# AVianEco/Softspoken

Measured on AMD Instinct MI355X. Metric: audio-seconds processed/sec (whole node), 16 kHz mono, higher is better.
Workload: dtype f16x2

## Files before the change

### softspoken_amd/build.py

```python
from __future__ import annotations

import os
import subprocess
import sys

HERE = os.path.dirname(os.path.abspath(__file__))
CSRC = os.path.join(HERE, "csrc")
OBJ = os.path.join(CSRC, "_obj")
LIB = os.path.join(HERE, "libsoftspoken_hip.so")
DEV_LIB = os.path.join(HERE, "libsoftspoken_hip_dev.so")
SOURCES = ["conv2.hip", "conv2_ups.hip", "conv4.hip", "conv4_ups.hip", "conv1s.hip", "conv9s.hip", "frontend.hip", "heads.hip", "weights.hip", "engine.hip", "host.hip", "abi.hip", "stream.hip", "separate.hip"]
HEADERS = [os.path.join(CSRC, h) for h in ("kernels.h", "engine.h", "dsp.h", "mfma_util.h", "conv4_forms.h", "stream16.h")] + [os.path.join(os.path.dirname(HERE), "include", "softspoken.h")]
FLAGS = ["-O3", "--offload-arch=gfx950", "-fPIC", "-std=c++17", "-Wno-unused-value"]
EXTRA_FLAGS = {"frontend.hip": ["-fno-slp-vectorize"], "conv4.hip": ["-fno-slp-vectorize"], "conv4_ups.hip": ["-fno-slp-vectorize"],
               "conv1s.hip": ["-fno-slp-vectorize"], "conv9s.hip": ["-fno-slp-vectorize"]}
DEV_SOURCES = ("conv2.hip", "conv2_ups.hip", "conv4.hip", "conv4_ups.hip", "conv1s.hip", "frontend.hip", "engine.hip", "weights.hip", "abi.hip", "separate.hip")
JITTER_LIB = DEV_LIB


def _hipcc():
    for cand in (os.environ.get("HIPCC"), "/opt/rocm/bin/hipcc"):
        if cand and os.path.exists(cand):
            return cand
    return "hipcc"


def _stale(target, deps):
    if not os.path.exists(target):
        return True
    t = os.path.getmtime(target)
    return any(os.path.getmtime(d) > t for d in deps)


def build(force: bool = False, verbose: bool = True, dev: bool = False, jitter: bool = False) -> str:
    dev = dev or jitter
    os.makedirs(OBJ, exist_ok=True)
    hipcc = _hipcc()
    objs, procs = [], []
# ... 28 lines not shown
```

### softspoken_amd/csrc/conv9s.hip

```cpp
#include "kernels.h"
#include "stream16.h"
#include <algorithm>

namespace ss {

static constexpr int kProjFrag = 2 * 2 * 2 * 1024;
static constexpr uint32_t kRowB = kW * 64, kRowB8 = (kW / 2) * 64;

__global__ __launch_bounds__(64 * kS1Waves) __attribute__((amdgpu_waves_per_eu(2, 2)))
void conv9_stream16_kernel(ConvArgs a, int rows_per_unit, int total_units) {
    extern __shared__ __attribute__((aligned(16))) char smem[];
    char* sW = smem;
    char* sP = smem + 2 * kBank;

    const int tid = threadIdx.x, lane = tid & 63, wave = __builtin_amdgcn_readfirstlane(tid >> 6);
    const int g = lane >> 4, c = lane & 15;
    for (int p = tid; p < 2 * kBank / 16; p += 64 * kS1Waves) *(u32x4*)(sW + p * 16) = *(const u32x4*)((const char*)a.wpk + (size_t)p * 16);
    for (int p = tid; p < kProjFrag / 16; p += 64 * kS1Waves) *(u32x4*)(sP + p * 16) = *(const u32x4*)((const char*)a.proj_w + (size_t)p * 16);
    const f32x4 bias[2] = {*(const f32x4*)(a.bias + 8 * g), *(const f32x4*)(a.bias + 8 * g + 4)};
    __syncthreads();

    const char* wl_base = sW + lane * 16;
    const char* pl_base = sP + lane * 16;
    const char* fw_base = (const char*)a.flat_w4 + lane * 16;
    const int bands = kH / rows_per_unit;
    const int64_t lo = a.lo_delta;
    uint32_t ovf = 0;

    for (int unit = (int)blockIdx.x * kS1Waves + wave; unit < total_units; unit += (int)gridDim.x * kS1Waves) {
        const int s = unit % kStrips, b = (unit / kStrips) % bands, n = unit / (kStrips * bands);
        const int x0 = kStripCols * s - 1, y0 = b * rows_per_unit, ylast = y0 + rows_per_unit - 1;
        uint32_t keep[2], voff[2]; bool st_lane[2];
        int xt[2];
#pragma unroll
        for (int t = 0; t < 2; ++t) {
            const int mm = 2 * c + t;
            xt[t] = x0 + mm;
            keep[t] = (unsigned)xt[t] < (unsigned)kW ? 0xffffffffu : 0u;
            st_lane[t] = mm >= 1 && mm <= kStripCols && xt[t] < kW;
            voff[t] = (uint32_t)min(max(xt[t], 0), kW - 1) * 64u + (uint32_t)g * 16u;
        }
        const uint32_t voff8 = (uint32_t)(min(max(xt[1], 0), kW - 1) >> 1) * 64u + (uint32_t)g * 16u;
        const char* hw = (const char*)a.src0 + (size_t)n * kH * kRowB;
        const char* c1w = (const char*)a.xp0 + (size_t)n * kH * kRowB;
        const char* c8w = (const char*)a.xp1 + (size_t)n * (kH / 2) * kRowB8;
        char* ow = (char*)a.out + (size_t)n * kH * kRowB;

        auto load_row = [&](S16Row& H, int r) {
            const char* p = hw + (size_t)min(max(r, 0), kH - 1) * kRowB;
#pragma unroll
            for (int t = 0; t < 2; ++t) { H.f[t][0] = *(const u32x4*)(p + voff[t]); H.f[t][1] = *(const u32x4*)(p + lo + voff[t]); }
        };
        auto mask_row = [&](S16Row& H, int r) {
            const uint32_t rk = (unsigned)r < (unsigned)kH ? 0xffffffffu : 0u;
#pragma unroll
            for (int t = 0; t < 2; ++t)
#pragma unroll
                for (int pq = 0; pq < 2; ++pq)
#pragma unroll
                    for (int e = 0; e < 4; ++e) H.f[t][pq][e] &= keep[t] & rk;
        };
        S16Row H0, H1, H2;
        S16Row C1;
        u32x4 C8[2];
        auto load_c1 = [&](int r) {
            const char* p = c1w + (size_t)r * kRowB;
#pragma unroll
            for (int t = 0; t < 2; ++t) { C1.f[t][0] = *(const u32x4*)(p + voff[t]); C1.f[t][1] = *(const u32x4*)(p + lo + voff[t]); }
        };
        auto load_c8 = [&](int r8) {
            const char* p = c8w + (size_t)r8 * kRowB8;
            C8[0] = *(const u32x4*)(p + voff8); C8[1] = *(const u32x4*)(p + lo + voff8);
        };
        f32x4 F[2] = {f32x4{0.f, 0.f, 0.f, 0.f}, f32x4{0.f, 0.f, 0.f, 0.f}};
        uint32_t ovt[2] = {0u, 0u};

        auto row_step = [&](int y, S16Row& Ha, const S16Row& Hb, S16Row& Hn) {
            S16Ring ring;
            ring.rd(wl_base, 0);
            u32x4 pw[2][2][2];
#pragma unroll
            for (int q = 0; q < 8; ++q) pw[q >> 2][(q >> 1) & 1][q & 1] = *(const u32x4*)(pl_base + q * 1024);
            const u32x4 fwh = *(const u32x4*)(fw_base + (size_t)(2 * y) * 1024), fwl = *(const u32x4*)(fw_base + (size_t)(2 * y + 1) * 1024);
            __builtin_amdgcn_sched_barrier(0);
            f32x4 P[3][2][2];
#pragma unroll
            for (int t = 0; t < 2; ++t)
#pragma unroll
                for (int u = 0; u < 2; ++u) { P[0][t][u] = f32x4{0.f, 0.f, 0.f, 0.f}; P[1][t][u] = bias[u]; P[2][t][u] = f32x4{0.f, 0.f, 0.f, 0.f}; }
            u32x4 c8t0[2];
#pragma unroll
            for (int pq = 0; pq < 2; ++pq)
#pragma unroll
                for (int e = 0; e < 4; ++e) c8t0[pq][e] = (uint32_t)s16_shr1((int)C8[pq][e]);
#pragma unroll
            for (int src = 0; src < 2; ++src)
#pragma unroll
                for (int pr = 0; pr < 3; ++pr)
#pragma unroll
                    for (int u = 0; u < 2; ++u)
#pragma unroll
                        for (int t = 0; t < 2; ++t) {
                            const int pq = pr == 0 ? 1 : 0;
                            const u32x4& x = src == 0 ? C1.f[t][pq] : (t ? C8[pq] : c8t0[pq]);
                            P[1][t][u] = s16_mfma(pw[src][u][pr == 1 ? 1 : 0], x, P[1][t][u]);
                        }
            __builtin_amdgcn_sched_barrier(0);
            load_c1(min(y + 1, ylast));
            load_c8(min(y + 1, ylast) >> 1);
            __builtin_amdgcn_sched_barrier(0);
            s16_taps(ring, wl_base, Ha, Hb, Hn, P, [&](int tap) {
                if (tap == 2) load_row(Ha, min(y + 2, ylast + 1));
                if (tap == 5) mask_row(Hn, y + 1);
            });
            float v[2][2][4];
            s16_combine(P, v);
            uint32_t kh[2][4], kl[2][4];
#pragma unroll
            for (int t = 0; t < 2; ++t) {
                s16_split_px(v[t], kh[t], kl[t]);
#pragma unroll
                for (int i = 0; i < 4; ++i) ovt[t] = pk_max_u16(ovt[t], kh[t][i]);
            }
#pragma unroll
            for (int pr = 0; pr < 3; ++pr)
#pragma unroll
                for (int t = 0; t < 2; ++t) {
                    const uint32_t (&k)[4] = pr == 0 ? kl[t] : kh[t];
                    F[t] = s16_mfma(pr == 1 ? fwl : fwh, u32x4{k[0], k[1], k[2], k[3]}, F[t]);
                }
            if (a.store_out) {
                char* p = ow + (size_t)y * kRowB;
#pragma unroll
                for (int t = 0; t < 2; ++t)
                    if (st_lane[t]) {
                        *(u32x4*)(p + voff[t]) = u32x4{kh[t][0], kh[t][1], kh[t][2], kh[t][3]};
                        *(u32x4*)(p + lo + voff[t]) = u32x4{kl[t][0], kl[t][1], kl[t][2], kl[t][3]};
                    }
            }
        };

        load_row(H0, y0 - 1); load_row(H1, y0); load_c1(y0); load_c8(y0 >> 1); load_row(H2, y0 + 1);
        mask_row(H0, y0 - 1); mask_row(H1, y0);
        int k = 0;
        for (; k + 3 <= rows_per_unit; k += 3) {
            row_step(y0 + k, H0, H1, H2);
            row_step(y0 + k + 1, H1, H2, H0);
            row_step(y0 + k + 2, H2, H0, H1);
        }
        if (k < rows_per_unit) {
            row_step(y0 + k, H0, H1, H2);
            if (k + 1 < rows_per_unit) row_step(y0 + k + 1, H1, H2, H0);
        }
#pragma unroll
        for (int t = 0; t < 2; ++t) {
            if (g == 0 && st_lane[t]) {
                float* fp = a.flat_part + ((size_t)n * bands + b) * 4 * kW + xt[t];
#pragma unroll
                for (int r = 0; r < 4; ++r) fp[r * kW] = F[t][r];
            }
            if (st_lane[t]) ovf = pk_max_u16(ovf, ovt[t]);
        }
    }
    if (((ovf & 0x7fff7fffu) + 0x04000400u) & 0x80008000u) atomicOr(a.range_flag, 1);
}

static bool px64(ActStride s) { return s.pix == 64u; }
bool conv9_stream_supports(const ConvArgs& a) {
    return a.H == kH && a.W == kW && a.Cout == kC && a.C0 == kC && a.C1 == 0 && a.C0x == kC && a.C1x == kC && a.src0 && a.xp0 && a.xp1 && a.wpk &&
           a.proj_w && a.bias && a.flat_w4 && a.flat_part && (a.out || !a.store_out) && !a.pool_out && !a.res_in && a.lo_delta != 0 && a.range_flag &&
           a.N > 0 && px64(a.s_src0) && px64(a.s_xp0) && px64(a.s_xp1) && (px64(a.s_out) || !a.store_out);
}
const char* conv9_stream_variant() { return "conv9_stream16_kernel"; }
size_t conv9_stream_proj_bytes() { return kProjFrag; }
size_t conv9_stream_flat_bytes() { return (size_t)kH * 2 * 1024; }
bool conv9_stream_rows_ok(int rows_per_unit) { return rows_per_unit >= 2 && !(rows_per_unit & 1) && kH % rows_per_unit == 0 && rows_per_unit <= kMaxRows; }
int conv9_stream_flat_groups(int rows_per_unit) { return kH / rows_per_unit; }
double conv9_stream_issued_macs(int N) { return (double)N * kH * kStrips * ((24 + 108 + 6) / 3) * (16.0 * 16 * 32); }

hipError_t launch_conv9_stream(const ConvArgs& a, int rows_per_unit, int grid_override, int num_cus, hipStream_t s) {
    if (!conv9_stream_supports(a) || !conv9_stream_rows_ok(rows_per_unit)) return hipErrorInvalidValue;
    const int64_t total = (int64_t)a.N * (kH / rows_per_unit) * kStrips;
    if (total >= (int64_t)1 << 30) return hipErrorInvalidValue;
    const int cus = num_cus > 0 ? num_cus : 256;
    int grid = (int)std::min<int64_t>(cus, (total + kS1Waves - 1) / kS1Waves);
    if (grid_override > 0) grid = std::min(grid, grid_override);
    static std::atomic<uint64_t> attr_done{0};
    const size_t lds = 2 * (size_t)kBank + kProjFrag;
    if (hipError_t e = allow_full_lds((const void*)conv9_stream16_kernel, attr_done)) return e;
    hipLaunchKernelGGL(conv9_stream16_kernel, dim3(grid), dim3(64 * kS1Waves), lds, s, a, rows_per_unit, (int)total);
    return hipGetLastError();
}

}
```

### softspoken_amd/csrc/engine.h

```cpp
#pragma once
#include "../../include/softspoken.h"
#include "kernels.h"

#include <map>
#include <set>
#include <string>
#include <vector>

namespace ss {

inline size_t pcm_bytes_per_sample(int format) {
    switch (format) {
        case SS_PCM_U8: case SS_PCM_S8: return 1;
        case SS_PCM_S16: case SS_PCM_S16BE: return 2;
        case SS_PCM_S24: case SS_PCM_S24BE: return 3;
        case SS_PCM_F64: case SS_PCM_F64BE: return 8;
        default: return 4;
    }
}

int fail(ss_ctx* c, int code, const std::string& msg);
const char* thread_error();

#define HIPCHK(c, expr)                                                                                   \
// ... 5 lines not shown

struct BlobEntry { char name[96]; uint32_t dtype, ndim; int64_t shape[4]; uint64_t offset, nbytes; };
static_assert(sizeof(BlobEntry) == 152, "blob entry layout");
struct Blob {
    std::map<std::string, BlobEntry> e;
    const char* base = nullptr;
    size_t size = 0;
    bool has(const std::string& k) const { return e.count(k) != 0; }
    const float* f32(const std::string& k, size_t count, std::string& err) const;
};
bool parse_blob(const void* p, size_t n, Blob& b, std::string& err);

enum Precision { kFp32 = 0, kBf16 = 1, kF16x2 = 2 };

struct ConvPlan {
    std::string name;
    void* d_w2 = nullptr; float* d_bias2 = nullptr; float* d_res_bias = nullptr; float* d_rank1 = nullptr;
    void* d_w3 = nullptr; void* d_proj = nullptr; float* d_bias3 = nullptr;
    void* d_w_ups = nullptr;
    bool s1_range_proven = false;
    void* d_w_s1 = nullptr;
    void* d_w_s16 = nullptr;
    void* d_proj_s16 = nullptr;
    void* d_w_upsr = nullptr;
    void* d_w_ups32 = nullptr;
    int ups32_nt = 1;
    int Cout = 0, NT = 1, C0 = 0, C1 = 0, R0 = 0, R1 = 0, H = 0, W = 0;
};

struct FileRec {
    int64_t off = 0;
    int64_t n = 0;
    int64_t n_padded = 0;
    double duration = 0;
    int64_t W = 0, win_base = 0;
    int64_t bin_off = 0; int n_bins = 0;
};

struct StreamSet;
struct SepState;

struct SepPlan {
    int N = 0, hop = 0;
    int64_t W = 0, n_bins = 0, windows_run = 0;
    std::vector<ss_separation_range> ranges;
};
// ... 170 lines not shown
```

### softspoken_amd/csrc/engine.hip

```cpp
#include "engine.h"

#include <algorithm>
#include <chrono>
#include <cmath>
#include <cstdio>
#include <cstdlib>
#include <cstring>

namespace ss {

static thread_local std::string g_err;

int fail(ss_ctx* c, int code, const std::string& msg) {
    g_err = msg;
    if (c) c->err = msg;
    return code;
}
const char* thread_error() { return g_err.c_str(); }

double now_ms() { return std::chrono::duration<double, std::milli>(std::chrono::steady_clock::now().time_since_epoch()).count(); }

static int stat_id(ss_ctx* c, const std::string& name) {
    for (size_t i = 0; i < c->stats.size(); ++i) if (c->stats[i].name == name) return (int)i;
    KStat k; k.name = name; c->stats.push_back(k);
// ... 262 lines not shown
    a.N = n; a.H = pa.H; a.W = pa.W; a.Cout = pa.Cout; a.C0 = pa.C0; a.C1 = pa.C1; a.relu = 1;
    b.src0 = h; b.wpk = pb.d_w2; b.bias = pb.d_bias3; b.out = out; b.pool_out = pool;
    b.N = n; b.H = pb.H; b.W = pb.W; b.Cout = pb.Cout; b.C0 = pb.Cout; b.C1 = 0; b.relu = 1;
    b.proj_w = pb.d_proj; b.xp0 = x0; b.xp1 = x1; b.C0x = pa.C0; b.C1x = pa.C1;
    b.flat_w4 = ex.flat_w4; b.flat_part = ex.flat_part; b.store_out = ex.store_out;
    a.dbg = b.dbg = base_dbg();
    if (!(stride_of(ws, x0, a.s_src0) && stride_of(ws, x1, a.s_src1) && stride_of(ws, h, a.s_out) && stride_of(ws, h, b.s_src0) &&
          stride_of(ws, out, b.s_out) && stride_of(ws, pool, b.s_pool)))
        return fail(c, SS_ERR_STATE, "no byte order for a tensor of " + pa.name);
    b.s_xp0 = a.s_src0; b.s_xp1 = a.s_src1;
    ConvArgs au = a;
    au.wpk = pa.d_w_ups;
    const bool ups = c->prec == kF16x2 && pa.d_w_ups && x1 && conv_ups_supports(au, cus);
    if ((!ups && !conv_v4_supports(a, pa.NT, cus, prec4)) || !conv_v4_supports(b, pb.NT, cus, prec4)) return 1;
    mark_written(c, ws, h); mark_written(c, ws, pool);
    if (ex.store_out) mark_written(c, ws, out);
    const double px = (double)n * pa.H * pa.W, cin = pa.C0 + pa.C1, cinb = pa.C0 + pa.C1 / 4.0;
    const double flops_a = 2.0 * px * pa.Cout * 9.0 * cin, bytes_a = px * es * (cinb + pa.Cout);
    auto v4 = [&](const ConvPlan& p, ConvArgs& x, double flops, double bytes) {
        return conv_launch(c, stream, conv_v4_variant(x, p.NT, cus, prec4), p.name, x, flops, bytes, -1.0,
                           [&](ConvArgs& y) { return launch_conv3x3_v4(y, p.NT, cus, prec4, stream); });
    };
    int rc;
    if (ups) {
        ScopedLaunch sl(c, stream, std::string(conv_ups_variant()) + "/" + pa.name, flops_a, bytes_a, px * pa.Cout * (9.0 * pa.C0 + 4.0 * pa.C1));
        HIPCHK(c, launch_conv3x3_ups(au, cus, stream));
    } else if ((rc = v4(pa, a, flops_a, bytes_a))) return rc;
    const double flops_b = 2.0 * px * pb.Cout * (9.0 * pb.Cout + cin) + (ex.flat_part ? 2.0 * px * 32 * 4 : 0.0);
    const double bytes_b = px * es * (pb.Cout + cinb + (ex.flat_part && !ex.store_out ? 0 : pb.Cout) + (pool ? pb.Cout / 4.0 : 0));
    if (c->prec == kF16x2 && ex.flat_part && ex.flat_rows && pb.d_w_s16 && pb.d_proj_s16 && dev_env("SOFTSPOKEN_C9S", 1)) {
        ConvArgs bs = b;
        bs.wpk = pb.d_w_s16; bs.proj_w = pb.d_proj_s16; bs.flat_w4 = ex.flat_rows;
        const int rows = dev_env("SOFTSPOKEN_C9S_ROWS", 32);
        if (conv9_stream_supports(bs) && conv9_stream_rows_ok(rows)) {
            const int grid = dev_env("SOFTSPOKEN_C9S_GRID", 0);
            if ((rc = conv_launch(c, stream, conv9_stream_variant(), pb.name, bs, flops_b, bytes_b, conv9_stream_issued_macs(n),
                                  [&](ConvArgs& y) { return launch_conv9_stream(y, rows, grid, cus, stream); })))
                return rc;
            ws.flat_groups = conv9_stream_flat_groups(rows);
            return SS_OK;
        }
    }
    if ((rc = v4(pb, b, flops_b, bytes_b))) return rc;
    if (ex.flat_part) ws.flat_groups = conv_v4_flat_groups();
    return SS_OK;
}

// ... 403 lines not shown
```

### softspoken_amd/csrc/kernels.h

```cpp
#pragma once
#include <hip/hip_runtime.h>
#include <stdint.h>
#include <atomic>
#include <cstdlib>

namespace ss {

#ifdef SS_DEVBUILD
static inline int dev_env(const char* name, int dflt) { const char* v = getenv(name); return v ? atoi(v) : dflt; }
#else
static constexpr int dev_env(const char*, int dflt) { return dflt; }
#endif

inline hipError_t allow_full_lds(const void* kernel, std::atomic<uint64_t>& done) {
    int dev = 0;
    hipError_t e = hipGetDevice(&dev);
    if (e != hipSuccess) return e;
    const uint64_t bit = 1ull << (dev & 63);
    if (done.load(std::memory_order_acquire) & bit) return hipSuccess;
    e = hipFuncSetAttribute(kernel, hipFuncAttributeMaxDynamicSharedMemorySize, 160 * 1024);
    if (e == hipSuccess) done.fetch_or(bit, std::memory_order_release);
    return e;
}

// ... 95 lines not shown
const char* conv_upsr_variant();
size_t conv_upsr_weight_bytes(int C0, int C1, int Cout);
hipError_t launch_conv3x3_upsr(const ConvArgs& a, int num_cus, hipStream_t s);

bool conv_ups32_supports(const ConvArgs& a, int NT, int MTW, int num_cus);
const char* conv_ups32_variant(int NT, int MTW);
size_t conv_ups32_weight_bytes(int C0, int C1, int Cout);
hipError_t launch_conv3x3_ups32(const ConvArgs& a, int NT, int MTW, int num_cus, hipStream_t s);

bool conv1_stream_supports(const ConvArgs& a);
const char* conv1_stream_variant(const ConvArgs& a, int form);
size_t conv1_stream_weight_bytes();
hipError_t launch_conv1_stream(const ConvArgs& a, int form, int rows_per_unit, int num_cus, hipStream_t s);

bool conv9_stream_supports(const ConvArgs& a);
const char* conv9_stream_variant();
size_t conv9_stream_proj_bytes();
size_t conv9_stream_flat_bytes();
bool conv9_stream_rows_ok(int rows_per_unit);
int conv9_stream_flat_groups(int rows_per_unit);
double conv9_stream_issued_macs(int N);
hipError_t launch_conv9_stream(const ConvArgs& a, int rows_per_unit, int grid_override, int num_cus, hipStream_t s);

struct Head1dWeights { float w1[4][4][3], b1[4], w2[4][4][3], wr[4][4], b2r[4], wo[4], bo, fscale; };
hipError_t launch_mask_head_parts(const float* parts, int n_parts, const float* flat_bias, const Head1dWeights& hw, float* logits,
                                  int N, hipStream_t s);
hipError_t launch_spec_tail(const void* x, int64_t lo_delta, const float* w , const float* bias, float* spec, int N, int prec,
                            hipStream_t s);

static constexpr int kMelLo = 10, kMelHi = 32, kMelPitch = 43;
struct FrontendTables {
    const float4* pretw;
    const float2* w2048;
    const int* mel_start;
    const int* mel_count;
    const int* mel_off;
    const float* mel_w;
    int mel_nw;
    const float* mel_wp;
    int dbg;
    const float2* win2;
    const float2* twt;
    const float2* wkt;
    const float* mel_wq;
    const int* mel_p0;
};
// ... 50 lines not shown
```

### softspoken_amd/csrc/stream16.h

```cpp
#pragma once
#include "mfma_util.h"

namespace ss {

static constexpr int kH = 128, kW = 256, kC = 32;
static constexpr int kStrips = 9, kStripCols = 30;
static constexpr int kBank = 9 * 2 * 1024;
static constexpr int kS1Waves = 8;
static constexpr int kMaxRows = 32;

struct S16Row { u32x4 f[2][2]; };

__device__ __forceinline__ f32x4 s16_mfma(const u32x4& a, const u32x4& b, const f32x4& c) {
    return __builtin_amdgcn_mfma_f32_16x16x32_f16(__builtin_bit_cast(f16x8, a), __builtin_bit_cast(f16x8, b), c, 0, 0, 0);
}
__device__ __forceinline__ int s16_shr1(int v) { return __builtin_amdgcn_update_dpp(0, v, 0x111, 0xf, 0xf, true); }
__device__ __forceinline__ int s16_shl1(int v) { return __builtin_amdgcn_update_dpp(0, v, 0x101, 0xf, 0xf, true); }
__device__ __forceinline__ float s16_shr1f(float v) { return __int_as_float(s16_shr1(__float_as_int(v))); }
__device__ __forceinline__ float s16_shl1f(float v) { return __int_as_float(s16_shl1(__float_as_int(v))); }

struct S16Ring {
    u32x4 wh[2][2], wl[2][2];
    __device__ __forceinline__ void rd(const char* wl_base, int tap) {
#pragma unroll
// ... 16 lines not shown
#pragma unroll
        for (int pr = 0; pr < 3; ++pr)
#pragma unroll
            for (int u = 0; u < 2; ++u)
#pragma unroll
                for (int t = 0; t < 2; ++t)
                    P[dx][t][u] = s16_mfma(pr == 1 ? ring.wl[tap & 1][u] : ring.wh[tap & 1][u], Hr.f[t][pr == 0 ? 1 : 0], P[dx][t][u]);
        __builtin_amdgcn_sched_barrier(0);
        if (tap + 1 < 9) after_tap(tap);
    }
    __builtin_amdgcn_sched_barrier(0);
}

__device__ __forceinline__ void s16_combine(const f32x4 (&P)[3][2][2], float (&v)[2][2][4]) {
#pragma unroll
    for (int u = 0; u < 2; ++u)
#pragma unroll
        for (int r = 0; r < 4; ++r) {
            v[0][u][r] = relu_i(P[1][0][u][r] + s16_shr1f(P[0][1][u][r]) + P[2][1][u][r]);
            v[1][u][r] = relu_i(P[1][1][u][r] + P[0][0][u][r] + s16_shl1f(P[2][0][u][r]));
        }
}

__device__ __forceinline__ void s16_split_px(const float (&val)[2][4], uint32_t (&kh)[4], uint32_t (&kl)[4]) {
#pragma unroll
    for (int i = 0; i < 4; ++i) {
        const float e0 = val[i >> 1][2 * (i & 1)], e1 = val[i >> 1][2 * (i & 1) + 1];
        kh[i] = pack_f16(e0, e1);
        kl[i] = split_lo(kh[i], e0, e1);
    }
}

}
```

### softspoken_amd/csrc/weights.hip

```cpp
#include "engine.h"

#include <algorithm>
#include <cmath>
#include <cstring>

namespace ss {

const float* Blob::f32(const std::string& k, size_t count, std::string& err) const {
    auto it = e.find(k);
    if (it == e.end()) { err = "weights blob: missing tensor '" + k + "'"; return nullptr; }
    if (it->second.dtype != 0 || it->second.nbytes != count * 4) {
        err = "weights blob: tensor '" + k + "' has wrong dtype/size"; return nullptr;
    }
    return (const float*)(base + it->second.offset);
}

bool parse_blob(const void* p, size_t n, Blob& b, std::string& err) {
    if (n < 16 || memcmp(p, "SSWBLOB1", 8) != 0) { err = "weights blob: bad magic"; return false; }
    uint32_t cnt; memcpy(&cnt, (const char*)p + 8, 4);
    if (16 + (size_t)cnt * sizeof(BlobEntry) > n) { err = "weights blob: truncated table"; return false; }
    b.base = (const char*)p; b.size = n;
    for (uint32_t i = 0; i < cnt; ++i) {
        BlobEntry en; memcpy(&en, (const char*)p + 16 + (size_t)i * sizeof(BlobEntry), sizeof(BlobEntry));
        en.name[95] = 0;
// ... 186 lines not shown
                for (int l = 0; l < 64; ++l)
                    for (int e = 0; e < 8; ++e) {
                        const int co = l & 31, k = ci * 32 + s * 16 + (l >> 5) * 8 + e;
                        const size_t off = (size_t)ci * 2 * bank_r + (size_t)t * 2048 + ((size_t)s * 64 + l) * 16 + (size_t)e * 2;
                        put(off, off + bank_r, w3.w[((size_t)co * w3.cin + k) * 9 + t]);
                    }
    static const int lo_of[2][2] = {{0, 1}, {0, 2}}, hi_of[2][2] = {{0, 2}, {1, 2}};
    for (int cu = 0; cu < nups; ++cu)
        for (int cls = 0; cls < 4; ++cls)
            for (int t = 0; t < 4; ++t)
                for (int s = 0; s < 2; ++s)
                    for (int l = 0; l < 64; ++l)
                        for (int e = 0; e < 8; ++e) {
                            const int a = cls & 1, b = cls >> 1, ty = t >> 1, tx = t & 1;
                            const int co = l & 31, k = c0 + cu * 32 + s * 16 + (l >> 5) * 8 + e;
                            double sum = 0.0;
                            for (int dy = lo_of[a][ty]; dy <= hi_of[a][ty]; ++dy)
                                for (int dx = lo_of[b][tx]; dx <= hi_of[b][tx]; ++dx) sum += (double)w3.w[((size_t)co * w3.cin + k) * 9 + dy * 3 + dx];
                            const size_t off = (size_t)nreg * 2 * bank_r + (size_t)cu * 2 * bank_u + ((size_t)cls * 4 + t) * 2048 + ((size_t)s * 64 + l) * 16 + (size_t)e * 2;
                            put(off, off + bank_u, (float)sum);
                        }
}

static void pack_conv_split_upsr(const Folded& w3, const Folded& wr, int c0, int c1, std::vector<char>& out, bool& range_ok) {
    const size_t ent_r = (size_t)10 * 2048, ent_rh = ent_r + 256, ent_u = (size_t)17 * 2048;
    const int nreg = c0 / 32, nups = c1 / 32, ngroups = w3.cout / 32;
    const size_t group = (size_t)nreg * (ent_rh + ent_r) + (size_t)nups * 2 * ent_u;
    out.assign((size_t)ngroups * group, 0);
    auto put = [&](size_t off_hi, size_t off_lo, float v) {
        const uint16_t hi = f2h(v), lo = f2h(v - h2f(hi));
        if ((hi & 0x7c00u) == 0x7c00u) range_ok = false;
        memcpy(&out[off_hi], &hi, 2); memcpy(&out[off_lo], &lo, 2);
    };
    static const int lo_of[2][2] = {{0, 1}, {0, 2}}, hi_of[2][2] = {{0, 2}, {1, 2}};
    for (int g = 0; g < ngroups; ++g) {
        const size_t gb = (size_t)g * group;
        for (int ci = 0; ci < nreg; ++ci) {
            const size_t eh = gb + (size_t)ci * (ent_rh + ent_r), el = eh + ent_rh;
            for (int t = 0; t < 10; ++t)
                for (int s = 0; s < 2; ++s)
                    for (int l = 0; l < 64; ++l)
                        for (int e = 0; e < 8; ++e) {
                            const int co = g * 32 + (l & 31), k = ci * 32 + s * 16 + (l >> 5) * 8 + e;
                            const float v = t < 9 ? w3.w[((size_t)co * w3.cin + k) * 9 + t] : wr.w[(size_t)co * wr.cin + k];
                            const size_t off = (size_t)t * 2048 + ((size_t)s * 64 + l) * 16 + (size_t)e * 2;
                            put(eh + off, el + off, v);
// ... 291 lines not shown
    }
    if (c->prec == kFp32 && cin1 >= 16 && cin0 % 16 == 0 && cin1 % 16 == 0 && cout % 32 == 0 && H % 16 == 0 && dev_env("SOFTSPOKEN_UPS32", 1)) {
        A.ups32_nt = dev_env("SOFTSPOKEN_UPS32_NT", 1);
        if (A.ups32_nt < 1 || A.ups32_nt > 3 || (cout / 32) % A.ups32_nt) A.ups32_nt = 1;
        pack_conv_v2_ups(f1, fr, cin0, cin1, A.ups32_nt, pk);
        if (pk.size() != conv_ups32_weight_bytes(cin0, cin1, cout)) return fail(c, SS_ERR_STATE, "pack_conv_v2_ups: size");
        if ((rc = dev_upload(c, (char**)&A.d_w_ups32, pk.data(), pk.size()))) return rc;
    }
    c->convs.push_back(A);
    if (c->bf16) {
        pack_conv_v2(f1, nullptr, true, NT, pk);
        if ((rc = dev_upload(c, (char**)&A.d_w3, pk.data(), pk.size()))) return rc;
        c->convs.back().d_w3 = A.d_w3;
    }
    if (c->prec == kF16x2) {
        pack_conv_split(f1, nullptr, NTA, pk, c->split_range_ok);
        if ((rc = dev_upload(c, (char**)&A.d_w3, pk.data(), pk.size()))) return rc;
        c->convs.back().d_w3 = A.d_w3;
        if (cin1 >= 32 && cin0 >= 32 && cout == 32) {
            pack_conv_split_ups(f1, cin0, cin1, pk, c->split_range_ok);
            if (pk.size() != conv_ups_weight_bytes(cin0, cin1)) return fail(c, SS_ERR_STATE, "pack_conv_split_ups: size");
            if ((rc = dev_upload(c, (char**)&A.d_w_ups, pk.data(), pk.size()))) return rc;
            c->convs.back().d_w_ups = A.d_w_ups;
        }
    }
    const int NTB = (c->prec == kF16x2 && NT == 3 && dev_env("SOFTSPOKEN_NTB1", 1)) ? 1 : NT;
    ConvPlan B; B.name = name + ".B"; B.Cout = cout; B.NT = NTB; B.C0 = cout; B.R0 = cin0; B.R1 = cin1; B.H = H; B.W = W;
    if (c->bf16 && cin % 16 == 0) {
        const int steps = cin / 16, tiles = cout / 32;
        std::vector<uint16_t> pj((size_t)steps * tiles * 64 * 8);
        for (int st = 0; st < steps; ++st) for (int t = 0; t < tiles; ++t) for (int l = 0; l < 64; ++l) for (int j = 0; j < 8; ++j)
            pj[(((size_t)st * tiles + t) * 64 + l) * 8 + j] = f2bf(fr.w[(size_t)(32 * t + (l & 31)) * cin + 16 * st + 8 * (l >> 5) + j]);
        if ((rc = dev_upload(c, (char**)&B.d_proj, (const char*)pj.data(), pj.size() * 2))) return rc;
        if ((rc = dev_upload(c, &B.d_bias3, b2r.data(), cout * 4))) return rc;
    }
    if (c->prec == kF16x2 && cin % 16 == 0) {
        const int steps = cin / 16, tiles = cout / 32;
        const size_t bank = (size_t)steps * tiles * 64 * 8;
        std::vector<uint16_t> pj(2 * bank);
        for (int st = 0; st < steps; ++st) for (int t = 0; t < tiles; ++t) for (int l = 0; l < 64; ++l) for (int j = 0; j < 8; ++j) {
            const float v = fr.w[(size_t)(32 * t + (l & 31)) * cin + 16 * st + 8 * (l >> 5) + j];
            const uint16_t hi = f2h(v);
            if ((hi & 0x7c00u) == 0x7c00u) c->split_range_ok = false;
            const size_t at = (((size_t)st * tiles + t) * 64 + l) * 8 + j;
            pj[at] = hi; pj[bank + at] = f2h(v - h2f(hi));
        }
// ... 142 lines not shown
```

Measured before the change: 33200.

## Add streaming 3x3+upsample conv kernel and switch conv9 to 32-column halo strips

Adds a new streaming kernel for the fused 3x3 conv with a 2x-upsampled second input. It keeps a three-row ring of activations in registers and uses DPP lane shifts with halo columns to form the horizontal taps. Upsampled contributions use pre-summed parity weights packed on the host, so each output parity needs fewer MFMAs. The existing conv9 stream kernel moves to non-overlapping 32-column strips with halo loads instead of overlapping strips with masked stores, which removes redundant edge compute but adds halo loads and DPP ops. The new path is on by default when shapes match.

```diff
diff --git a/softspoken_amd/build.py b/softspoken_amd/build.py
--- a/softspoken_amd/build.py
+++ b/softspoken_amd/build.py
@@ -9,11 +9,11 @@
 OBJ = os.path.join(CSRC, "_obj")
 LIB = os.path.join(HERE, "libsoftspoken_hip.so")
 DEV_LIB = os.path.join(HERE, "libsoftspoken_hip_dev.so")
-SOURCES = ["conv2.hip", "conv2_ups.hip", "conv4.hip", "conv4_ups.hip", "conv1s.hip", "conv9s.hip", "frontend.hip", "heads.hip", "weights.hip", "engine.hip", "host.hip", "abi.hip", "stream.hip", "separate.hip"]
+SOURCES = ["conv2.hip", "conv2_ups.hip", "conv4.hip", "conv4_ups.hip", "conv1s.hip", "conv9s.hip", "conv9a.hip", "frontend.hip", "heads.hip", "weights.hip", "engine.hip", "host.hip", "abi.hip", "stream.hip", "separate.hip"]
 HEADERS = [os.path.join(CSRC, h) for h in ("kernels.h", "engine.h", "dsp.h", "mfma_util.h", "conv4_forms.h", "stream16.h")] + [os.path.join(os.path.dirname(HERE), "include", "softspoken.h")]
 FLAGS = ["-O3", "--offload-arch=gfx950", "-fPIC", "-std=c++17", "-Wno-unused-value"]
 EXTRA_FLAGS = {"frontend.hip": ["-fno-slp-vectorize"], "conv4.hip": ["-fno-slp-vectorize"], "conv4_ups.hip": ["-fno-slp-vectorize"],
-               "conv1s.hip": ["-fno-slp-vectorize"], "conv9s.hip": ["-fno-slp-vectorize"]}
+               "conv1s.hip": ["-fno-slp-vectorize"], "conv9s.hip": ["-fno-slp-vectorize"], "conv9a.hip": ["-fno-slp-vectorize"]}
 DEV_SOURCES = ("conv2.hip", "conv2_ups.hip", "conv4.hip", "conv4_ups.hip", "conv1s.hip", "frontend.hip", "engine.hip", "weights.hip", "abi.hip", "separate.hip")
 JITTER_LIB = DEV_LIB
 
diff --git a/softspoken_amd/csrc/conv9a.hip b/softspoken_amd/csrc/conv9a.hip
--- /dev/null
+++ b/softspoken_amd/csrc/conv9a.hip
@@ -0,0 +1,164 @@
+#include "kernels.h"
+#include "stream16.h"
+#include <algorithm>
+#include <type_traits>
+
+namespace ss {
+
+static constexpr int kUpsFrag = 2 * 2 * 4 * 2 * 2 * 1024;
+static constexpr uint32_t kRowB = kW * 64, kRowB8 = (kW / 2) * 64;
+
+struct A9Row8 { u32x4 f[2]; u32x4 h[2]; };
+
+__global__ __launch_bounds__(64 * kS1Waves) __attribute__((amdgpu_waves_per_eu(2, 2)))
+void conv3x3_ups_stream16_kernel(ConvArgs a, int rows_per_unit, int total_units) {
+    extern __shared__ __attribute__((aligned(16))) char smem[];
+    char* sW = smem;
+    char* sU = smem + 2 * kBank;
+
+    const int tid = threadIdx.x, lane = tid & 63, wave = __builtin_amdgcn_readfirstlane(tid >> 6);
+    const int g = lane >> 4, c = lane & 15;
+    for (int p = tid; p < 2 * kBank / 16; p += 64 * kS1Waves) *(u32x4*)(sW + p * 16) = *(const u32x4*)((const char*)a.wpk + (size_t)p * 16);
+    for (int p = tid; p < kUpsFrag / 16; p += 64 * kS1Waves) *(u32x4*)(sU + p * 16) = *(const u32x4*)((const char*)a.wpk_b + (size_t)p * 16);
+    const f32x4 bias[2] = {*(const f32x4*)(a.bias + 8 * g), *(const f32x4*)(a.bias + 8 * g + 4)};
+    __syncthreads();
+
+    const char* wl_base = sW + lane * 16;
+    const char* ul_base = sU + lane * 16;
+    const int bands = kH / rows_per_unit;
+    const int64_t lo = a.lo_delta;
+    uint32_t ovf = 0;
+
+    for (int unit = (int)blockIdx.x * kS1Waves + wave; unit < total_units; unit += (int)gridDim.x * kS1Waves) {
+        const int s = unit % kStrips32, b = (unit / kStrips32) % bands, n = unit / (kStrips32 * bands);
+        const int x0 = 32 * s, y0 = b * rows_per_unit, ylast = y0 + rows_per_unit - 1;
+        const uint32_t voff[2] = {(uint32_t)(x0 + 2 * c) * 64u + (uint32_t)g * 16u, (uint32_t)(x0 + 2 * c + 1) * 64u + (uint32_t)g * 16u};
+        const uint32_t hoff = (uint32_t)(c < 8 ? max(x0 - 1, 0) : min(x0 + 32, kW - 1)) * 64u + (uint32_t)g * 16u;
+        const uint32_t voff8 = (uint32_t)(x0 / 2 + c) * 64u + (uint32_t)g * 16u;
+        const uint32_t hoff8 = (uint32_t)(c < 8 ? max(x0 / 2 - 1, 0) : min(x0 / 2 + 16, kW / 2 - 1)) * 64u + (uint32_t)g * 16u;
+        const uint32_t hkeep = (c < 8 ? s > 0 : s < kStrips32 - 1) ? 0xffffffffu : 0u;
+        const char* c1w = (const char*)a.src0 + (size_t)n * kH * kRowB;
+        const char* c8w = (const char*)a.src1 + (size_t)n * (kH / 2) * kRowB8;
+        char* ow = (char*)a.out + (size_t)n * kH * kRowB;
+
+        auto load_row = [&](S16RowH& H, int r) {
+            const char* p = c1w + (size_t)min(max(r, 0), kH - 1) * kRowB;
+#pragma unroll
+            for (int t = 0; t < 2; ++t) { H.f[t][0] = *(const u32x4*)(p + voff[t]); H.f[t][1] = *(const u32x4*)(p + lo + voff[t]); }
+            H.h[0] = *(const u32x4*)(p + hoff); H.h[1] = *(const u32x4*)(p + lo + hoff);
+        };
+        auto mask_row = [&](S16RowH& H, int r) {
+            const uint32_t rk = (unsigned)r < (unsigned)kH ? 0xffffffffu : 0u;
+#pragma unroll
+            for (int pq = 0; pq < 2; ++pq)
+#pragma unroll
+                for (int e = 0; e < 4; ++e) { H.f[0][pq][e] &= rk; H.f[1][pq][e] &= rk; H.h[pq][e] &= hkeep & rk; }
+        };
+        auto load_row8 = [&](A9Row8& K, int r8) {
+            const char* p = c8w + (size_t)min(max(r8, 0), kH / 2 - 1) * kRowB8;
+            K.f[0] = *(const u32x4*)(p + voff8); K.f[1] = *(const u32x4*)(p + lo + voff8);
+            K.h[0] = *(const u32x4*)(p + hoff8); K.h[1] = *(const u32x4*)(p + lo + hoff8);
+        };
+        auto mask_row8 = [&](A9Row8& K, int r8) {
+            const uint32_t rk = (unsigned)r8 < (unsigned)(kH / 2) ? 0xffffffffu : 0u;
+#pragma unroll
+            for (int pq = 0; pq < 2; ++pq)
+#pragma unroll
+                for (int e = 0; e < 4; ++e) { K.f[pq][e] &= rk; K.h[pq][e] &= hkeep & rk; }
+        };
+        S16RowH H0, H1, H2;
+        A9Row8 K0, K1, K2;
+        S16Ring3 ring;
+        uint32_t ovt = 0;
+
+        auto row_step = [&](auto parity, int y, S16RowH& Ha, const S16RowH& Hb, S16RowH& Hn, A9Row8& Ka, const A9Row8& Kb, A9Row8& Kc) {
+            constexpr int par = decltype(parity)::value;
+            auto form = [](int q) { return ((q & 1) << 1) | ((q >> 1) & 1); };
+            auto rd_set8 = [&](int q) {
+                const char* p = ul_base + (((par * 2 + (q >> 2)) * 4 + form(q)) * 4) * 1024;
+                ring.rd((q + 1) % 3, p, p + 1024, 2048);
+            };
+            f32x4 P[2][2];
+#pragma unroll
+            for (int t = 0; t < 2; ++t)
+#pragma unroll
+                for (int u = 0; u < 2; ++u) P[t][u] = bias[u];
+            s16_taps_shifted(ring, wl_base, Ha, Hb, Hn, P, [&] { rd_set8(0); rd_set8(1); }, [&](int tap) {
+                if (tap == 2) load_row(Ha, min(y + 2, ylast + 1));
+                if (tap == 5) { mask_row(Hn, y + 1); if constexpr (par != 0) mask_row8(Kc, (y >> 1) + 1); }
+            });
+#pragma unroll
+            for (int q = 0; q < 8; ++q) {
+                const int ty = q >> 2, f = form(q), t = f >> 1, slot = (q + 1) % 3;
+                const A9Row8& K = par == 0 ? (ty == 0 ? Ka : Kb) : (ty == 0 ? Kb : Kc);
+                if (q + 2 < 8) rd_set8(q + 2);
+                else if (q == 6) ring.rd_tap(0, wl_base, 0);
+                u32x4 B[2];
+#pragma unroll
+                for (int pq = 0; pq < 2; ++pq) B[pq] = f == 0 ? s16_shr1_halo(K.f[pq], K.h[pq]) : (f == 3 ? s16_shl1_halo(K.f[pq], K.h[pq]) : K.f[pq]);
+                __builtin_amdgcn_sched_barrier(0);
+                s16_products(ring, slot, B, P[t]);
+                __builtin_amdgcn_sched_barrier(0);
+                if (par == 0 && q == 3) load_row8(Ka, min((y >> 1) + 2, (ylast >> 1) + 1));
+            }
+            char* p = ow + (size_t)y * kRowB;
+#pragma unroll
+            for (int t = 0; t < 2; ++t) {
+                float v[2][4];
+#pragma unroll
+                for (int u = 0; u < 2; ++u)
+#pragma unroll
+                    for (int r = 0; r < 4; ++r) v[u][r] = relu_i(P[t][u][r]);
+                uint32_t kh[4], kl[4];
+                s16_split_px(v, kh, kl);
+#pragma unroll
+                for (int i = 0; i < 4; ++i) ovt = pk_max_u16(ovt, kh[i]);
+                *(u32x4*)(p + voff[t]) = u32x4{kh[0], kh[1], kh[2], kh[3]};
+                *(u32x4*)(p + lo + voff[t]) = u32x4{kl[0], kl[1], kl[2], kl[3]};
+            }
+        };
+
+        load_row(H0, y0 - 1); load_row(H1, y0); load_row8(K0, (y0 >> 1) - 1); load_row8(K1, y0 >> 1); load_row(H2, y0 + 1); load_row8(K2, (y0 >> 1) + 1);
+        ring.rd_tap(0, wl_base, 0);
+        mask_row(H0, y0 - 1); mask_row(H1, y0); mask_row8(K0, (y0 >> 1) - 1); mask_row8(K1, y0 >> 1);
+        const std::integral_constant<int, 0> even; const std::integral_constant<int, 1> odd;
+        for (int k = 0; k < rows_per_unit; k += 6) {
+            row_step(even, y0 + k, H0, H1, H2, K0, K1, K2);
+            row_step(odd, y0 + k + 1, H1, H2, H0, K0, K1, K2);
+            if (k + 2 >= rows_per_unit) break;
+            row_step(even, y0 + k + 2, H2, H0, H1, K1, K2, K0);
+            row_step(odd, y0 + k + 3, H0, H1, H2, K1, K2, K0);
+            if (k + 4 >= rows_per_unit) break;
+            row_step(even, y0 + k + 4, H1, H2, H0, K2, K0, K1);
+            row_step(odd, y0 + k + 5, H2, H0, H1, K2, K0, K1);
+        }
+        ovf = pk_max_u16(ovf, ovt);
+    }
+    if (((ovf & 0x7fff7fffu) + 0x04000400u) & 0x80008000u) atomicOr(a.range_flag, 1);
+}
+
+static bool px64(ActStride s) { return s.pix == 64u; }
+bool conv9a_stream_supports(const ConvArgs& a) {
+    return a.plain && a.H == kH && a.W == kW && a.Cout == kC && a.C0 == kC && a.C1 == kC && a.src0 && a.src1 && a.wpk && a.wpk_b && a.bias && a.out &&
+           !a.pool_out && !a.res_in && !a.res_out && a.lo_delta != 0 && a.range_flag && a.N > 0 && px64(a.s_src0) && px64(a.s_src1) && px64(a.s_out);
+}
+const char* conv9a_stream_variant() { return "conv3x3_ups_stream16_kernel"; }
+size_t conv9a_stream_ups_bytes() { return kUpsFrag; }
+bool conv9a_stream_rows_ok(int rows_per_unit) { return rows_per_unit >= 2 && !(rows_per_unit & 1) && kH % rows_per_unit == 0 && rows_per_unit <= kMaxRows; }
+double conv9a_stream_issued_macs(int N) { return (double)N * kH * kStrips32 * ((108 + 48) / 3) * (16.0 * 16 * 32); }
+
+hipError_t launch_conv9a_stream(const ConvArgs& a, int rows_per_unit, int grid_override, int num_cus, hipStream_t s) {
+    if (!conv9a_stream_supports(a) || !conv9a_stream_rows_ok(rows_per_unit)) return hipErrorInvalidValue;
+    const int64_t total = (int64_t)a.N * (kH / rows_per_unit) * kStrips32;
+    if (total >= (int64_t)1 << 30) return hipErrorInvalidValue;
+    const int cus = num_cus > 0 ? num_cus : 256;
+    int grid = (int)std::min<int64_t>(cus, (total + kS1Waves - 1) / kS1Waves);
+    if (grid_override > 0) grid = std::min(grid, grid_override);
+    static std::atomic<uint64_t> attr_done{0};
+    const size_t lds = 2 * (size_t)kBank + kUpsFrag;
+    if (hipError_t e = allow_full_lds((const void*)conv3x3_ups_stream16_kernel, attr_done)) return e;
+    hipLaunchKernelGGL(conv3x3_ups_stream16_kernel, dim3(grid), dim3(64 * kS1Waves), lds, s, a, rows_per_unit, (int)total);
+    return hipGetLastError();
+}
+
+}
diff --git a/softspoken_amd/csrc/conv9s.hip b/softspoken_amd/csrc/conv9s.hip
--- a/softspoken_amd/csrc/conv9s.hip
+++ b/softspoken_amd/csrc/conv9s.hip
@@ -28,39 +28,32 @@
     uint32_t ovf = 0;
 
     for (int unit = (int)blockIdx.x * kS1Waves + wave; unit < total_units; unit += (int)gridDim.x * kS1Waves) {
-        const int s = unit % kStrips, b = (unit / kStrips) % bands, n = unit / (kStrips * bands);
-        const int x0 = kStripCols * s - 1, y0 = b * rows_per_unit, ylast = y0 + rows_per_unit - 1;
-        uint32_t keep[2], voff[2]; bool st_lane[2];
-        int xt[2];
-#pragma unroll
-        for (int t = 0; t < 2; ++t) {
-            const int mm = 2 * c + t;
-            xt[t] = x0 + mm;
-            keep[t] = (unsigned)xt[t] < (unsigned)kW ? 0xffffffffu : 0u;
-            st_lane[t] = mm >= 1 && mm <= kStripCols && xt[t] < kW;
-            voff[t] = (uint32_t)min(max(xt[t], 0), kW - 1) * 64u + (uint32_t)g * 16u;
-        }
-        const uint32_t voff8 = (uint32_t)(min(max(xt[1], 0), kW - 1) >> 1) * 64u + (uint32_t)g * 16u;
+        const int s = unit % kStrips32, b = (unit / kStrips32) % bands, n = unit / (kStrips32 * bands);
+        const int x0 = 32 * s, y0 = b * rows_per_unit, ylast = y0 + rows_per_unit - 1;
+        const int xt[2] = {x0 + 2 * c, x0 + 2 * c + 1};
+        const uint32_t voff[2] = {(uint32_t)xt[0] * 64u + (uint32_t)g * 16u, (uint32_t)xt[1] * 64u + (uint32_t)g * 16u};
+        const uint32_t hoff = (uint32_t)(c < 8 ? max(x0 - 1, 0) : min(x0 + 32, kW - 1)) * 64u + (uint32_t)g * 16u;
+        const uint32_t hkeep = (c < 8 ? s > 0 : s < kStrips32 - 1) ? 0xffffffffu : 0u;
+        const uint32_t voff8 = (uint32_t)(x0 / 2 + c) * 64u + (uint32_t)g * 16u;
         const char* hw = (const char*)a.src0 + (size_t)n * kH * kRowB;
         const char* c1w = (const char*)a.xp0 + (size_t)n * kH * kRowB;
         const char* c8w = (const char*)a.xp1 + (size_t)n * (kH / 2) * kRowB8;
         char* ow = (char*)a.out + (size_t)n * kH * kRowB;
 
-        auto load_row = [&](S16Row& H, int r) {
+        auto load_row = [&](S16RowH& H, int r) {
             const char* p = hw + (size_t)min(max(r, 0), kH - 1) * kRowB;
 #pragma unroll
             for (int t = 0; t < 2; ++t) { H.f[t][0] = *(const u32x4*)(p + voff[t]); H.f[t][1] = *(const u32x4*)(p + lo + voff[t]); }
+            H.h[0] = *(const u32x4*)(p + hoff); H.h[1] = *(const u32x4*)(p + lo + hoff);
         };
-        auto mask_row = [&](S16Row& H, int r) {
+        auto mask_row = [&](S16RowH& H, int r) {
             const uint32_t rk = (unsigned)r < (unsigned)kH ? 0xffffffffu : 0u;
 #pragma unroll
-            for (int t = 0; t < 2; ++t)
+            for (int pq = 0; pq < 2; ++pq)
 #pragma unroll
-                for (int pq = 0; pq < 2; ++pq)
-#pragma unroll
-                    for (int e = 0; e < 4; ++e) H.f[t][pq][e] &= keep[t] & rk;
+                for (int e = 0; e < 4; ++e) { H.f[0][pq][e] &= rk; H.f[1][pq][e] &= rk; H.h[pq][e] &= hkeep & rk; }
         };
-        S16Row H0, H1, H2;
+        S16RowH H0, H1, H2;
         S16Row C1;
         u32x4 C8[2];
         auto load_c1 = [&](int r) {
@@ -75,24 +68,19 @@
         f32x4 F[2] = {f32x4{0.f, 0.f, 0.f, 0.f}, f32x4{0.f, 0.f, 0.f, 0.f}};
         uint32_t ovt[2] = {0u, 0u};
 
-        auto row_step = [&](int y, S16Row& Ha, const S16Row& Hb, S16Row& Hn) {
-            S16Ring ring;
-            ring.rd(wl_base, 0);
+        auto row_step = [&](int y, S16RowH& Ha, const S16RowH& Hb, S16RowH& Hn) {
+            S16Ring3 ring;
+            ring.rd_tap(0, wl_base, 0);
             u32x4 pw[2][2][2];
 #pragma unroll
             for (int q = 0; q < 8; ++q) pw[q >> 2][(q >> 1) & 1][q & 1] = *(const u32x4*)(pl_base + q * 1024);
             const u32x4 fwh = *(const u32x4*)(fw_base + (size_t)(2 * y) * 1024), fwl = *(const u32x4*)(fw_base + (size_t)(2 * y + 1) * 1024);
             __builtin_amdgcn_sched_barrier(0);
-            f32x4 P[3][2][2];
+            f32x4 P[2][2];
 #pragma unroll
             for (int t = 0; t < 2; ++t)
 #pragma unroll
-                for (int u = 0; u < 2; ++u) { P[0][t][u] = f32x4{0.f, 0.f, 0.f, 0.f}; P[1][t][u] = bias[u]; P[2][t][u] = f32x4{0.f, 0.f, 0.f, 0.f}; }
-            u32x4 c8t0[2];
-#pragma unroll
-            for (int pq = 0; pq < 2; ++pq)
-#pragma unroll
-                for (int e = 0; e < 4; ++e) c8t0[pq][e] = (uint32_t)s16_shr1((int)C8[pq][e]);
+                for (int u = 0; u < 2; ++u) P[t][u] = bias[u];
 #pragma unroll
             for (int src = 0; src < 2; ++src)
 #pragma unroll
@@ -102,19 +90,25 @@
 #pragma unroll
                         for (int t = 0; t < 2; ++t) {
                             const int pq = pr == 0 ? 1 : 0;
-                            const u32x4& x = src == 0 ? C1.f[t][pq] : (t ? C8[pq] : c8t0[pq]);
-                            P[1][t][u] = s16_mfma(pw[src][u][pr == 1 ? 1 : 0], x, P[1][t][u]);
+                            const u32x4& x = src == 0 ? C1.f[t][pq] : C8[pq];
+                            P[t][u] = s16_mfma(pw[src][u][pr == 1 ? 1 : 0], x, P[t][u]);
                         }
             __builtin_amdgcn_sched_barrier(0);
             load_c1(min(y + 1, ylast));
             load_c8(min(y + 1, ylast) >> 1);
             __builtin_amdgcn_sched_barrier(0);
-            s16_taps(ring, wl_base, Ha, Hb, Hn, P, [&](int tap) {
+            s16_taps_shifted(ring, wl_base, Ha, Hb, Hn, P, [] {}, [&](int tap) {
                 if (tap == 2) load_row(Ha, min(y + 2, ylast + 1));
                 if (tap == 5) mask_row(Hn, y + 1);
             });
+            __builtin_amdgcn_sched_barrier(0);
             float v[2][2][4];
-            s16_combine(P, v);
+#pragma unroll
+            for (int t = 0; t < 2; ++t)
+#pragma unroll
+                for (int u = 0; u < 2; ++u)
+#pragma unroll
+                    for (int r = 0; r < 4; ++r) v[t][u][r] = relu_i(P[t][u][r]);
             uint32_t kh[2][4], kl[2][4];
 #pragma unroll
             for (int t = 0; t < 2; ++t) {
@@ -132,11 +126,10 @@
             if (a.store_out) {
                 char* p = ow + (size_t)y * kRowB;
 #pragma unroll
-                for (int t = 0; t < 2; ++t)
-                    if (st_lane[t]) {
-                        *(u32x4*)(p + voff[t]) = u32x4{kh[t][0], kh[t][1], kh[t][2], kh[t][3]};
-                        *(u32x4*)(p + lo + voff[t]) = u32x4{kl[t][0], kl[t][1], kl[t][2], kl[t][3]};
-                    }
+                for (int t = 0; t < 2; ++t) {
+                    *(u32x4*)(p + voff[t]) = u32x4{kh[t][0], kh[t][1], kh[t][2], kh[t][3]};
+                    *(u32x4*)(p + lo + voff[t]) = u32x4{kl[t][0], kl[t][1], kl[t][2], kl[t][3]};
+                }
             }
         };
 
@@ -154,12 +147,12 @@
         }
 #pragma unroll
         for (int t = 0; t < 2; ++t) {
-            if (g == 0 && st_lane[t]) {
+            if (g == 0) {
                 float* fp = a.flat_part + ((size_t)n * bands + b) * 4 * kW + xt[t];
 #pragma unroll
                 for (int r = 0; r < 4; ++r) fp[r * kW] = F[t][r];
             }
-            if (st_lane[t]) ovf = pk_max_u16(ovf, ovt[t]);
+            ovf = pk_max_u16(ovf, ovt[t]);
         }
     }
     if (((ovf & 0x7fff7fffu) + 0x04000400u) & 0x80008000u) atomicOr(a.range_flag, 1);
@@ -176,11 +169,11 @@
 size_t conv9_stream_flat_bytes() { return (size_t)kH * 2 * 1024; }
 bool conv9_stream_rows_ok(int rows_per_unit) { return rows_per_unit >= 2 && !(rows_per_unit & 1) && kH % rows_per_unit == 0 && rows_per_unit <= kMaxRows; }
 int conv9_stream_flat_groups(int rows_per_unit) { return kH / rows_per_unit; }
-double conv9_stream_issued_macs(int N) { return (double)N * kH * kStrips * ((24 + 108 + 6) / 3) * (16.0 * 16 * 32); }
+double conv9_stream_issued_macs(int N) { return (double)N * kH * kStrips32 * ((24 + 108 + 6) / 3) * (16.0 * 16 * 32); }
 
 hipError_t launch_conv9_stream(const ConvArgs& a, int rows_per_unit, int grid_override, int num_cus, hipStream_t s) {
     if (!conv9_stream_supports(a) || !conv9_stream_rows_ok(rows_per_unit)) return hipErrorInvalidValue;
-    const int64_t total = (int64_t)a.N * (kH / rows_per_unit) * kStrips;
+    const int64_t total = (int64_t)a.N * (kH / rows_per_unit) * kStrips32;
     if (total >= (int64_t)1 << 30) return hipErrorInvalidValue;
     const int cus = num_cus > 0 ? num_cus : 256;
     int grid = (int)std::min<int64_t>(cus, (total + kS1Waves - 1) / kS1Waves);
diff --git a/softspoken_amd/csrc/engine.h b/softspoken_amd/csrc/engine.h
--- a/softspoken_amd/csrc/engine.h
+++ b/softspoken_amd/csrc/engine.h
@@ -51,6 +51,7 @@
     void* d_w_s1 = nullptr;
     void* d_w_s16 = nullptr;
     void* d_proj_s16 = nullptr;
+    void* d_w_a16 = nullptr; void* d_w_ups16 = nullptr;
     void* d_w_upsr = nullptr;
     void* d_w_ups32 = nullptr;
     int ups32_nt = 1;
diff --git a/softspoken_amd/csrc/engine.hip b/softspoken_amd/csrc/engine.hip
--- a/softspoken_amd/csrc/engine.hip
+++ b/softspoken_amd/csrc/engine.hip
@@ -308,7 +308,15 @@
                            [&](ConvArgs& y) { return launch_conv3x3_v4(y, p.NT, cus, prec4, stream); });
     };
     int rc;
-    if (ups) {
+    ConvArgs as = a;
+    as.wpk = pa.d_w_a16; as.wpk_b = pa.d_w_ups16;
+    const int rows_a = dev_env("SOFTSPOKEN_C9A_ROWS", 32);
+    if (ups && pa.d_w_a16 && pa.d_w_ups16 && dev_env("SOFTSPOKEN_C9A", 1) && conv9a_stream_supports(as) && conv9a_stream_rows_ok(rows_a)) {
+        const int grid = dev_env("SOFTSPOKEN_C9A_GRID", 0);
+        if ((rc = conv_launch(c, stream, conv9a_stream_variant(), pa.name, as, flops_a, bytes_a, conv9a_stream_issued_macs(n),
+                              [&](ConvArgs& y) { return launch_conv9a_stream(y, rows_a, grid, cus, stream); })))
+            return rc;
+    } else if (ups) {
         ScopedLaunch sl(c, stream, std::string(conv_ups_variant()) + "/" + pa.name, flops_a, bytes_a, px * pa.Cout * (9.0 * pa.C0 + 4.0 * pa.C1));
         HIPCHK(c, launch_conv3x3_ups(au, cus, stream));
     } else if ((rc = v4(pa, a, flops_a, bytes_a))) return rc;
diff --git a/softspoken_amd/csrc/kernels.h b/softspoken_amd/csrc/kernels.h
--- a/softspoken_amd/csrc/kernels.h
+++ b/softspoken_amd/csrc/kernels.h
@@ -141,6 +141,13 @@
 double conv9_stream_issued_macs(int N);
 hipError_t launch_conv9_stream(const ConvArgs& a, int rows_per_unit, int grid_override, int num_cus, hipStream_t s);
 
+bool conv9a_stream_supports(const ConvArgs& a);
+const char* conv9a_stream_variant();
+size_t conv9a_stream_ups_bytes();
+bool conv9a_stream_rows_ok(int rows_per_unit);
+double conv9a_stream_issued_macs(int N);
+hipError_t launch_conv9a_stream(const ConvArgs& a, int rows_per_unit, int grid_override, int num_cus, hipStream_t s);
+
 struct Head1dWeights { float w1[4][4][3], b1[4], w2[4][4][3], wr[4][4], b2r[4], wo[4], bo, fscale; };
 hipError_t launch_mask_head_parts(const float* parts, int n_parts, const float* flat_bias, const Head1dWeights& hw, float* logits,
                                   int N, hipStream_t s);
diff --git a/softspoken_amd/csrc/stream16.h b/softspoken_amd/csrc/stream16.h
--- a/softspoken_amd/csrc/stream16.h
+++ b/softspoken_amd/csrc/stream16.h
@@ -62,6 +62,66 @@
         }
 }
 
+static constexpr int kStrips32 = 8;
+
+struct S16RowH { u32x4 f[2][2]; u32x4 h[2]; };
+
+__device__ __forceinline__ u32x4 s16_shr1_halo(const u32x4& v, const u32x4& halo) {
+    u32x4 r;
+#pragma unroll
+    for (int e = 0; e < 4; ++e) r[e] = (uint32_t)__builtin_amdgcn_update_dpp((int)halo[e], (int)v[e], 0x111, 0xf, 0xf, false);
+    return r;
+}
+__device__ __forceinline__ u32x4 s16_shl1_halo(const u32x4& v, const u32x4& halo) {
+    u32x4 r;
+#pragma unroll
+    for (int e = 0; e < 4; ++e) r[e] = (uint32_t)__builtin_amdgcn_update_dpp((int)halo[e], (int)v[e], 0x101, 0xf, 0xf, false);
+    return r;
+}
+
+struct S16Ring3 {
+    u32x4 wh[3][2], wl[3][2];
+    __device__ __forceinline__ void rd(int slot, const char* hi, const char* lo, int step) {
+#pragma unroll
+        for (int u = 0; u < 2; ++u) { wh[slot][u] = *(const u32x4*)(hi + u * step); wl[slot][u] = *(const u32x4*)(lo + u * step); }
+    }
+    __device__ __forceinline__ void rd_tap(int slot, const char* wl_base, int tap) { rd(slot, wl_base + tap * 2048, wl_base + kBank + tap * 2048, 1024); }
+};
+
+__device__ __forceinline__ void s16_products(const S16Ring3& ring, int slot, const u32x4 (&B)[2], f32x4 (&Pt)[2]) {
+#pragma unroll
+    for (int pr = 0; pr < 3; ++pr)
+#pragma unroll
+        for (int u = 0; u < 2; ++u) Pt[u] = s16_mfma(pr == 1 ? ring.wl[slot][u] : ring.wh[slot][u], B[pr == 0 ? 1 : 0], Pt[u]);
+}
+
+template <typename Last, typename AfterTap>
+__device__ __forceinline__ void s16_taps_shifted(S16Ring3& ring, const char* wl_base, const S16RowH& Ha, const S16RowH& Hb, const S16RowH& Hn,
+                                                 f32x4 (&P)[2][2], Last&& before_last, AfterTap&& after_tap) {
+#pragma unroll
+    for (int tap = 0; tap < 9; ++tap) {
+        const int dy = tap / 3, dx = tap % 3 - 1, slot = tap & 1;
+        const S16RowH& Hr = dy == 0 ? Ha : (dy == 1 ? Hb : Hn);
+        if (tap + 1 < 9) ring.rd_tap(slot ^ 1, wl_base, tap + 1); else before_last();
+        u32x4 B[2][2];
+#pragma unroll
+        for (int pq = 0; pq < 2; ++pq) {
+            B[0][pq] = dx == 0 ? Hr.f[0][pq] : (dx < 0 ? s16_shr1_halo(Hr.f[1][pq], Hr.h[pq]) : Hr.f[1][pq]);
+            B[1][pq] = dx == 0 ? Hr.f[1][pq] : (dx < 0 ? Hr.f[0][pq] : s16_shl1_halo(Hr.f[0][pq], Hr.h[pq]));
+        }
+        __builtin_amdgcn_sched_barrier(0);
+#pragma unroll
+        for (int pr = 0; pr < 3; ++pr)
+#pragma unroll
+            for (int u = 0; u < 2; ++u)
+#pragma unroll
+                for (int t = 0; t < 2; ++t)
+                    P[t][u] = s16_mfma(pr == 1 ? ring.wl[slot][u] : ring.wh[slot][u], B[t][pr == 0 ? 1 : 0], P[t][u]);
+        __builtin_amdgcn_sched_barrier(0);
+        after_tap(tap);
+    }
+}
+
 __device__ __forceinline__ void s16_split_px(const float (&val)[2][4], uint32_t (&kh)[4], uint32_t (&kl)[4]) {
 #pragma unroll
     for (int i = 0; i < 4; ++i) {
diff --git a/softspoken_amd/csrc/weights.hip b/softspoken_amd/csrc/weights.hip
--- a/softspoken_amd/csrc/weights.hip
+++ b/softspoken_amd/csrc/weights.hip
@@ -232,6 +232,27 @@
                         }
 }
 
+static void pack_ups_stream16(const Folded& w3, int c0, std::vector<char>& out, bool& range_ok) {
+    out.assign((size_t)2 * 2 * 4 * 2 * 2 * 1024, 0);
+    static const int lo_of[2][2] = {{0, 1}, {0, 2}}, hi_of[2][2] = {{0, 2}, {1, 2}};
+    for (int a = 0; a < 2; ++a)
+        for (int ty = 0; ty < 2; ++ty)
+            for (int f = 0; f < 4; ++f)
+                for (int u = 0; u < 2; ++u)
+                    for (int l = 0; l < 64; ++l)
+                        for (int j = 0; j < 8; ++j) {
+                            const int b = f >> 1, tx = f & 1, i = l & 15, co = 8 * (i >> 2) + 4 * u + (i & 3), ci = c0 + 8 * (l >> 4) + j;
+                            double sum = 0.0;
+                            for (int dy = lo_of[a][ty]; dy <= hi_of[a][ty]; ++dy)
+                                for (int dx = lo_of[b][tx]; dx <= hi_of[b][tx]; ++dx) sum += (double)w3.w[((size_t)co * w3.cin + ci) * 9 + dy * 3 + dx];
+                            const float v = (float)sum;
+                            const uint16_t hi = f2h(v), lo = f2h(v - h2f(hi));
+                            if ((hi & 0x7c00u) == 0x7c00u) range_ok = false;
+                            const size_t off = ((size_t)((((a * 2 + ty) * 4 + f) * 2 + u) * 2) * 64 + l) * 16 + (size_t)j * 2;
+                            memcpy(&out[off], &hi, 2); memcpy(&out[off + 1024], &lo, 2);
+                        }
+}
+
 static void pack_conv_split_upsr(const Folded& w3, const Folded& wr, int c0, int c1, std::vector<char>& out, bool& range_ok) {
     const size_t ent_r = (size_t)10 * 2048, ent_rh = ent_r + 256, ent_u = (size_t)17 * 2048;
     const int nreg = c0 / 32, nups = c1 / 32, ngroups = w3.cout / 32;
@@ -569,6 +590,15 @@
             if (pk.size() != conv_ups_weight_bytes(cin0, cin1)) return fail(c, SS_ERR_STATE, "pack_conv_split_ups: size");
             if ((rc = dev_upload(c, (char**)&A.d_w_ups, pk.data(), pk.size()))) return rc;
             c->convs.back().d_w_ups = A.d_w_ups;
+            if (cin0 == 32 && cin1 == 32 && H == 128 && W == 256) {
+                pack_conv_stream16(f1, pk, c->split_range_ok);
+                if (pk.size() != conv1_stream_weight_bytes()) return fail(c, SS_ERR_STATE, "pack_conv_stream16: size");
+                if ((rc = dev_upload(c, (char**)&A.d_w_a16, pk.data(), pk.size()))) return rc;
+                pack_ups_stream16(f1, cin0, pk, c->split_range_ok);
+                if (pk.size() != conv9a_stream_ups_bytes()) return fail(c, SS_ERR_STATE, "pack_ups_stream16: size");
+                if ((rc = dev_upload(c, (char**)&A.d_w_ups16, pk.data(), pk.size()))) return rc;
+                c->convs.back().d_w_a16 = A.d_w_a16; c->convs.back().d_w_ups16 = A.d_w_ups16;
+            }
         }
     }
     const int NTB = (c->prec == kF16x2 && NT == 3 && dev_env("SOFTSPOKEN_NTB1", 1)) ? 1 : NT;
```

New measurement: 34130 (median of 6 runs). 1.03x the previous value.
